# Zain-Jiang/Speech-Editing-Toolkit

Measured on AMD Instinct MI355X. Metric: diffusion mel-frames/s (100-step p_sample, B=32/GPU, T=800), higher is better.
Workload: dtype f32 (operands carried as 2 fp16 pieces, 3 MFMA products per term, fp32 accumulate: fp32-equivalent, see roofline.note)

## Files before the change

include/set_amd.h:

```cpp
#ifndef SET_AMD_H
#define SET_AMD_H

#include <stdint.h>

#ifdef __cplusplus
extern "C" {
#endif

#define SET_AMD_ABI_VERSION 2

#define SET_OK 0
#define SET_E_INVALID (-1)
#define SET_E_UNSUPPORTED (-2)
#define SET_E_LAUNCH (-3)

#define SET_ACT_NONE 0
#define SET_ACT_RELU 1
#define SET_ACT_GELU 2
#define SET_ACT_TANH 3
#define SET_ACT_SOFTPLUS 4
#define SET_ACT_MISH 5
#define SET_ACT_LRELU 6

#define SET_PRO_NONE 0
// ... 236 lines not shown
    uint16_t *y16;
    uint16_t *z16;
    int64_t d_bs, d_cs;
    int32_t B, T, dil, first;
} SetDiffnetLayerBf16Args;
int64_t set_sizeof_diffnet_layer_bf16_args(void);
int64_t set_diffnet_layer_bf16_image_size(void);
int set_pack_diffnet_layer_bf16(const float *wdil , const float *wcond ,
                                const float *wout , void *img, void *stream);
int set_pack_diffnet_layers_bf16(const float *wdil, const float *wcond, const float *wout, int64_t sdil, int64_t scond, int64_t sout,
                                 void *img, int32_t L, void *stream);
int set_diffnet_layer_fwd_bf16(const SetDiffnetLayerBf16Args *args, void *stream);
typedef struct SetDiffnetLayersBf16Args {
    const float *x_in;
    float *x_out;
    float *skip;
    const float *cond;
    const float *dstep;
    const void *img;
    const float *b_dil, *b_cond, *b_out;
    float *scratch;
    int64_t scratch_floats;
    int64_t d_bs, d_cs, d_ls;
    int32_t B, T, l0, nl, dilation_cycle_length, first;
} SetDiffnetLayersBf16Args;
int64_t set_sizeof_diffnet_layers_bf16_args(void);
int64_t set_diffnet_layers_bf16_scratch_floats(int32_t B, int32_t T, int32_t l0, int32_t nl, int32_t dilation_cycle_length);
int32_t set_diffnet_layers_bf16_plan(int32_t B, int32_t T, int32_t L, int32_t dilation_cycle_length);
int set_diffnet_layers_fwd_bf16(const SetDiffnetLayersBf16Args *args, void *stream);
int set_debug_bf16_phase_buffer(uint64_t *buf);
int set_debug_split_phase_buffer(uint64_t *buf);
int set_debug_x3_phase_buffer(uint64_t *buf);
int set_debug_resblock_phase_buffer(uint64_t *buf);

typedef struct SetDiffnetLayerBf16BwdArgs {
    const float *dx_out;
    const float *dskip;
    const uint16_t *y16;
    const void *img;
    float *dx;
    uint16_t *dy16;
    uint16_t *do16;
    float *dcond;
    float *part_dbo;
    float *part_dby;
    float *part_dd;
    int32_t B, T, dil, dcond_first;
} SetDiffnetLayerBf16BwdArgs;
int64_t set_sizeof_diffnet_layer_bf16_bwd_args(void);
int32_t set_diffnet_layer_bwd_bf16_tiles(int32_t T, int32_t dil);
int set_diffnet_layer_bwd_bf16(const SetDiffnetLayerBf16BwdArgs *args, void *stream);
int set_diffnet_layer_bwd_reduce(const float *part_dbo, const float *part_dby, const float *part_dd, int32_t B, int32_t tiles,
                                 float *db_out, float *db_dil, float *db_cond, float *dd, int64_t dd_bs, void *stream);
int set_diffnet_layers_bwd_reduce(const float *part_dbo, const float *part_dby, const float *part_dd, int32_t B, int32_t tiles, int32_t L,
                                  float *db_out, int64_t s_out, float *db_dil, int64_t s_dil, float *db_cond, int64_t s_cond, float *dd,
                                  int64_t dd_bs, int64_t dd_ls, void *stream);
int set_partial_rows_sum(const float *part, float *out, int32_t groups, int32_t rows, int32_t cols, int32_t accumulate,
                         float scale, void *stream);

int set_step_proj_fwd(const float *h, const float *w, int64_t w_ls, const float *b, int64_t b_ls, float *out, int32_t L, int32_t C,
                      int32_t N, void *stream);
int64_t set_step_proj_bwd_scratch_floats(int32_t L, int32_t C, int32_t N);
int set_step_proj_bwd(const float *h, const float *g, const float *w, int64_t w_ls, float *dh, float *dw, int64_t dw_ls, float *db,
                      int64_t db_ls, float *scratch, int32_t L, int32_t C, int32_t N, void *stream);
int set_step_proj_bwd_dh(const float *g, const float *w, int64_t w_ls, float *dh, float *scratch, int32_t L, int32_t C, int32_t N,
                         void *stream);
// ... 144 lines not shown
```

speech-editing-toolkit_amd/_lib.py:

```python
import ctypes as C
import os
import shutil
import subprocess

_PKG = os.path.dirname(os.path.abspath(__file__))
_ROOT = os.path.dirname(_PKG)
CSRC = os.path.join(_PKG, "csrc")
INCLUDE = os.path.join(_ROOT, "include")
LIB_PATH = os.path.join(_PKG, "libset_amd.so")
_LIB_OVERRIDE = os.environ.get("SET_AMD_LIB")
SOURCES = ["conv1d.hip", "conv_x2.hip", "resblock_x2.hip", "glue.hip", "diffnet.hip", "diffnet_x3.hip", "boundary.hip", "diffusion_ops.hip", "diffusion_loop.hip",
           "train.hip", "attention.hip", "attention_fused.hip", "bf16.hip", "diffnet_bf16.hip", "stutter.hip"]
HIPCC_FLAGS = ["--offload-arch=gfx950", "-O3", "-std=c++17", "-fPIC", "-shared", "-ffp-contract=off"]

OK, E_INVALID, E_UNSUPPORTED, E_LAUNCH = 0, -1, -2, -3
ACT = dict(none=0, relu=1, gelu=2, tanh=3, softplus=4, mish=5, lrelu=6)
PRO = dict(none=0, lrelu=1, div=2)
IMPL_NAIVE, IMPL_MFMA, IMPL_MFMA2, IMPL_BF16, IMPL_F16X2, IMPL_FEWOUT = 1, 2, 3, 4, 5, 6
DTYPE_F32, DTYPE_BF16, DTYPE_BF16_G16, DTYPE_BF16_G16_X16 = 0, 1, 2, 3

c_f32p = C.POINTER(C.c_float)
c_i64p = C.POINTER(C.c_int64)


# ... 231 lines not shown
    "set_conv1d_wgrad": (C.c_int, [_V, _V, _V, _V, _I32, _I32, _I32, _I32, _I32, _I32, _I32, _I32, _I32, _F, _I32, _V]),
    "set_conv1d_wgrad_scratch_floats": (_I64, [_I32, _I32, _I32, _I32, _I32, _I32]),
    "set_conv1d_wgrad_det": (C.c_int, [_V, _V, _V, _V, _I32, _I32, _I32, _I32, _I32, _I32, _I32, _I32, _I32, _F, _I32, _V, _I64, _V]),
    "set_conv1d_wgrad_grouped_scratch_floats": (_I64, [_I32, _I32, _I32, _I32, _I32, _I32]),
    "set_conv1d_wgrad_det_grouped": (C.c_int, [_V, _V, _V, _V, _I32, _I64, _I64, _I64, _I64, _I32, _I32, _I32, _I32, _I32, _I32, _I32, _I32,
                                               _I32, _V, _I64, _V]),
    "set_packed_conv_weight_bf16_size": (_I64, [_I32, _I32, _I32]),
    "set_pack_conv_weight_bf16": (C.c_int, [_V, _V, _I32, _I32, _I32, _I64, _I64, _I64, _I64, _V]),
    "set_sizeof_pack_bf16_desc": (_I64, []),
    "set_pack_conv_weights_bf16_batch": (C.c_int, [_V, _I32, _I64, _V]),
    "set_sizeof_pack_f32_desc": (_I64, []),
    "set_fill_pack_f32_desc": (_I64, [C.POINTER(SetPackF32Desc), _I32, _I32]),
    "set_pack_conv_weights_f32_batch": (C.c_int, [_V, _I32, _I64, _V]),
    "set_channel_sum_det": (C.c_int, [_V, _V, _I32, _I32, _I32, _V, _V]),
    "set_weighted_sum_det": (C.c_int, [_V, _V, _V, _I64, _I64, _V, _V]),
    "set_sumsq_det": (C.c_int, [_V, _V, _I64, _V, _V]),
    "set_dur_loss_sums_det": (C.c_int, [_V, _V, _V, _V, _V, _I32, _I32, _I32, _I32, _V, _V]),
    "set_pitch_loss_sums_det": (C.c_int, [_V, _V, _V, _V, _V, _I32, _I32, _V, _V]),
    "set_scatter_rows_segments": (_I32, [_I32]),
    "set_scatter_rows_det": (C.c_int, [_V, _V, _V, _I32, _I32, _I32, _I32, _F, _I32, _I32, _V, _V]),
    "set_sizeof_diffnet_layer_bf16_args": (_I64, []),
    "set_diffnet_layer_bf16_image_size": (_I64, []),
    "set_pack_diffnet_layer_bf16": (C.c_int, [_V, _V, _V, _V, _V]),
    "set_pack_diffnet_layers_bf16": (C.c_int, [_V, _V, _V, _I64, _I64, _I64, _V, _I32, _V]),
    "set_diffnet_layer_fwd_bf16": (C.c_int, [C.POINTER(SetDiffnetLayerBf16Args), _V]),
    "set_sizeof_diffnet_layers_bf16_args": (_I64, []),
    "set_diffnet_layers_bf16_scratch_floats": (_I64, [_I32, _I32, _I32, _I32, _I32]),
    "set_diffnet_layers_fwd_bf16": (C.c_int, [C.POINTER(SetDiffnetLayersBf16Args), _V]),
    "set_diffnet_layers_bf16_plan": (_I32, [_I32, _I32, _I32, _I32]),
    "set_debug_bf16_phase_buffer": (C.c_int, [_V]),
    "set_debug_split_phase_buffer": (C.c_int, [_V]),
    "set_debug_x3_phase_buffer": (C.c_int, [_V]),
    "set_debug_resblock_phase_buffer": (C.c_int, [_V]),
    "set_sizeof_diffnet_layer_bf16_bwd_args": (_I64, []),
    "set_diffnet_layer_bwd_bf16_tiles": (_I32, [_I32, _I32]),
    "set_diffnet_layer_bwd_bf16": (C.c_int, [C.POINTER(SetDiffnetLayerBf16BwdArgs), _V]),
    "set_partial_rows_sum": (C.c_int, [_V, _V, _I32, _I32, _I32, _I32, _F, _V]),
    "set_step_proj_fwd": (C.c_int, [_V, _V, _I64, _V, _I64, _V, _I32, _I32, _I32, _V]),
    "set_step_proj_bwd_scratch_floats": (_I64, [_I32, _I32, _I32]),
    "set_step_proj_bwd": (C.c_int, [_V, _V, _V, _I64, _V, _V, _I64, _V, _I64, _V, _I32, _I32, _I32, _V]),
    "set_step_proj_bwd_dh": (C.c_int, [_V, _V, _I64, _V, _V, _I32, _I32, _I32, _V]),
    "set_step_proj_bwd_dw": (C.c_int, [_V, _V, _V, _I64, _V, _I64, _I32, _I32, _I32, _V]),
    "set_diffnet_layer_bwd_reduce": (C.c_int, [_V, _V, _V, _I32, _I32, _V, _V, _V, _V, _I64, _V]),
    "set_diffnet_layers_bwd_reduce": (C.c_int, [_V, _V, _V, _I32, _I32, _I32, _V, _I64, _V, _I64, _V, _I64, _V, _I64, _I64, _V]),
    "set_channel_sum": (C.c_int, [_V, _V, _I32, _I32, _I32, _V]),
    "set_row_sum": (C.c_int, [_V, _V, _I64, _I32, _F, _V]),
    "set_conv_epilogue_bwd": (C.c_int, [_V, _V, _V, _V, _I32, _I32, _I32, _I32, _F, _V]),
    "set_act_fwd": (C.c_int, [_V, _V, _I64, _I32, _F, _V]),
    "set_act_bwd": (C.c_int, [_V, _V, _V, _I64, _I32, _F, _V]),
    "set_act_bwd_scaled": (C.c_int, [_V, _V, _V, _I64, _I32, _F, _F, _V]),
    "set_gate_bwd": (C.c_int, [_V, _V, _V, _I32, _I32, _I32, _V]),
    "set_res_skip_bwd": (C.c_int, [_V, _V, _V, _V, _I32, _I32, _I32, _V]),
    "set_layernorm_ch_bwd": (C.c_int, [_V, _V, _V, _V, _V, _V, _V, _V, _I32, _I32, _I32, _F, _V]),
    "set_layernorm_ch_bwd_add": (C.c_int, [_V, _V, _V, _V, _V, _V, _V, _V, _V, _I32, _I32, _I32, _F, _V]),
    "set_layernorm_ch_bwd_scratch": (C.c_int64, [_I32, _I32, _I32]),
    "set_embedding_bwd": (C.c_int, [_V, _V, _V, _I32, _I32, _I32, _I32, _F, _I32, _V]),
    "set_expand_states_bwd": (C.c_int, [_V, _V, _V, _I32, _I32, _I32, _I32, _V]),
    "set_dropout": (C.c_int, [_V, _V, _I64, _F, _U64, _U64, _V]),
    "set_residual_dropout": (C.c_int, [_V, _V, _V, _V, _I32, _I32, _I32, _F, _U64, _U64, _V]),
    "set_conv_epilogue_bwd_dropout": (C.c_int, [_V, _V, _V, _V, _I32, _I32, _I32, _F, _U64, _U64, _V]),
    "set_stutter_head_scratch_floats": (_I64, [_I32, _I32, _I32]),
    "set_stutter_head_loss": (C.c_int, [_V, _V, _V, _V, _V, _V, _V, _I32, _I32, _I32, _V]),
    "set_stutter_head_loss_bwd": (C.c_int, [_V, _V, _V, _V, _V, _V, _V, _V, _V, _V, _V, _I32, _I32, _I32, _V]),
    "set_stutter_head_bwd_reduce": (C.c_int, [_V, _V, _V, _I32, _I32, _I32, _V]),
    "set_frame_weight": (C.c_int, [_V, _V, _I64, _I32, _V]),
    "set_weighted_sum": (C.c_int, [_V, _V, _V, _I64, _I64, _V]),
# ... 114 lines not shown
```

speech-editing-toolkit_amd/csrc/boundary.hip:

```cpp
#include <stdlib.h>

#include "common.h"
#include "boundary_x2.h"
#include "diffnet_host.h"

namespace {
constexpr int DC = 256;
}

struct BoundaryArgs {
    const float *skip;
    float *x;
    const float *eps;
    const float *coef4;
    const float *w_skip_p, *b_skip, *w_outp_p, *b_outp, *w_in_p, *b_in;
    float *xin_next;
    float inv_div;
    float div;
    uint64_t seed, quad_offset;
    int T, M, MP;
};
constexpr int BD_LD = 64;

__global__ void __launch_bounds__(256, 2) diffnet_boundary_kernel(BoundaryArgs a) {
// ... 101 lines not shown
        const float *bp = smem + half * BD_LD + l31;
        gemm_groups<1, 2, 4>(acc[i], wp, bp, 2 * BD_LD, (a.MP / 2) / 4, [&](int) {
            wp += 4 * 64;
            bp += 4 * 2 * BD_LD;
        });
    }
    const rsrc_t ro = make_rsrc(a.xin_next + (int64_t)b * DC * T);
    float bin[2][16];
#pragma unroll
    for (int i = 0; i < 2; ++i)
#pragma unroll
        for (int r = 0; r < 16; ++r) bin[i][r] = (a.b_in + 32 * (2 * w + i) + urow16(r))[4 * half];
#pragma unroll
    for (int cb = 0; cb < 2; ++cb) {
        if (t0 + 32 * cb + l31 < T) {
            const unsigned so = 4u * (unsigned)(4 * half * T + t0 + 32 * cb + l31);
#pragma unroll
            for (int i = 0; i < 2; ++i)
#pragma unroll
                for (int r = 0; r < 16; ++r) {
                    const int ur = 32 * (2 * w + i) + urow16(r);
                    buf_store(fmaxf(acc[i][0][cb][r] + bin[i][r], 0.0f), ro, so, 4u * (unsigned)ur * (unsigned)T);
                }
        }
    }
}

struct BoundaryX2Args {
    BoundaryArgs g;
    const unsigned short *w_skip_x2, *w_outp_x2, *w_in_x2;
    int32_t *err_flag;
};

__global__ void __launch_bounds__(256, 2) diffnet_boundary_x2_kernel(BoundaryX2Args ax) {
    const BoundaryArgs &a = ax.g;
    extern __shared__ __attribute__((aligned(16))) unsigned char bl[];
    const int tid = threadIdx.x, lane = tid & 63;
    const int w = __builtin_amdgcn_readfirstlane(tid >> 6);
    const int half = lane >> 5, l31 = lane & 31;
    const int b = blockIdx.y, t0 = blockIdx.x * 64, T = a.T, M = a.M;
    const unsigned lane16 = 16u * (unsigned)lane;
    const unsigned T4 = 4u * (unsigned)T;
    float amax = 0.0f;
    {
        const int f = lane, cg = w;
        const rsrc_t rs = make_rsrc(a.skip + (int64_t)b * DC * T);
        const unsigned vo = 4u * (unsigned)min(t0 + f, T - 1);
        const bool tv = t0 + f < T;
        for (int c0 = 0; c0 < 64; c0 += 16) {
            float v[16];
#pragma unroll
            for (int u = 0; u < 16; ++u) v[u] = buf_load(rs, vo, (unsigned)(64 * cg + c0 + u) * T4);
#pragma unroll
            for (int q8 = 0; q8 < 2; ++q8) {
                bx_u32x4 u0, u1;
#pragma unroll
                for (int e = 0; e < 4; ++e) {
                    unsigned short p0[2], p1[2];
#pragma unroll
                    for (int k = 0; k < 2; ++k) {
                        const float sv = v[8 * q8 + 2 * e + k] / a.div;
                        const float x = tv ? sv : 0.0f;
                        amax = fmaxf(amax, fabsf(x));
                        bx_split(x, p0[k], p1[k]);
                    }
                    u0[e] = (unsigned)p0[0] | ((unsigned)p0[1] << 16);
                    u1[e] = (unsigned)p1[0] | ((unsigned)p1[1] << 16);
                }
                *reinterpret_cast<bx_u32x4 *>(bl + f * BX_XR + (64 * cg + c0 + 8 * q8) * 2) = u0;
                *reinterpret_cast<bx_u32x4 *>(bl + BX_PIECE + f * BX_XR + (64 * cg + c0 + 8 * q8) * 2) = u1;
            }
        }
    }
    __syncthreads();
    auto bfrag256 = [&](int ks, int cb) { return (unsigned)((cb * 32 + l31) * BX_XR + (ks * 16 + half * 8) * 2); };
    {
        const rsrc_t rw = make_rsrc(ax.w_skip_x2);
        const float inv = reinterpret_cast<const float *>(ax.w_skip_x2 + (DC / 32) * (DC / 16) * 1024)[1];
        f32x16 acc[2][2];
#pragma unroll
        for (int i = 0; i < 2; ++i)
#pragma unroll
            for (int cb = 0; cb < 2; ++cb) acc[i][cb] = (f32x16){0};
        bx_gemm<2>(acc, rw, lane16, 2 * w, DC / 16, DC / 16, bl, BX_PIECE, bfrag256);
        __syncthreads();
#pragma unroll
        for (int i = 0; i < 2; ++i)
#pragma unroll
            for (int cb = 0; cb < 2; ++cb)
#pragma unroll
                for (int g = 0; g < 4; ++g) {
                    unsigned short p0[4], p1[4];
#pragma unroll
                    for (int e = 0; e < 4; ++e) {
                        const int row = 32 * (2 * w + i) + 8 * g + 4 * half + e;
                        const float h = fmaxf(acc[i][cb][4 * g + e] * inv + a.b_skip[row], 0.0f);
                        amax = fmaxf(amax, h);
                        bx_split(h, p0[e], p1[e]);
                    }
                    const unsigned off = (unsigned)((cb * 32 + l31) * BX_XR + (32 * (2 * w + i) + 8 * g + 4 * half) * 2);
                    bx_u32x2 u;
                    u[0] = (unsigned)p0[0] | ((unsigned)p0[1] << 16); u[1] = (unsigned)p0[2] | ((unsigned)p0[3] << 16);
                    *reinterpret_cast<bx_u32x2 *>(bl + off) = u;
                    u[0] = (unsigned)p1[0] | ((unsigned)p1[1] << 16); u[1] = (unsigned)p1[2] | ((unsigned)p1[3] << 16);
                    *reinterpret_cast<bx_u32x2 *>(bl + BX_PIECE + off) = u;
                }
    }
    __syncthreads();
    float *xs = reinterpret_cast<float *>(bl);
    {
        const int rbn = (M + 31) / 32;
        f32x16 xo[1][2];
        xo[0][0] = (f32x16){0};
        xo[0][1] = (f32x16){0};
        const float inv = reinterpret_cast<const float *>(ax.w_outp_x2 + ((M + 31) / 32) * (DC / 16) * 1024)[1];
        if (w < rbn) bx_gemm<1>(xo, make_rsrc(ax.w_outp_x2), lane16, w, DC / 16, DC / 16, bl, BX_PIECE, bfrag256);
        __syncthreads();
        if (w < 3) {
#pragma unroll
            for (int r = 0; r < 16; ++r) {
                const int row = 32 * w + mfma32_row(r, lane);
                const float bias = a.b_outp[min(row, M - 1)];
#pragma unroll
                for (int cb = 0; cb < 2; ++cb) xs[row * 64 + 32 * cb + l31] = (w < rbn && row < M) ? xo[0][cb][r] * inv + bias : 0.0f;
            }
        }
    }
    __syncthreads();
    {
        const float c1 = a.coef4[0], c2 = a.coef4[1], sig = a.coef4[3] * expf(0.5f * a.coef4[2]);
        float *xb = a.x + (int64_t)b * M * T;
        const float *eb = a.eps ? a.eps + (int64_t)b * M * T : nullptr;
        for (int qi = tid; qi < 96 * 16; qi += 256) {
            const int m = qi >> 4, tq = qi & 15, t = t0 + 4 * tq;
            float *cell = xs + m * 64 + 4 * tq;
            if (m < M && t < T) {
                const int64_t i = (int64_t)m * T + t;
                const f32x4 xt = *reinterpret_cast<const f32x4 *>(xb + i);
                float z[4];
                if (eb) {
                    const f32x4 e4 = *reinterpret_cast<const f32x4 *>(eb + i);
                    z[0] = e4[0]; z[1] = e4[1]; z[2] = e4[2]; z[3] = e4[3];
                } else {
                    randn4(a.seed, a.quad_offset + (uint64_t)(((int64_t)b * M * T + i) >> 2), z);
                }
                f32x4 o;
#pragma unroll
                for (int k = 0; k < 4; ++k) {
                    const float mean = c1 * cell[k] + c2 * xt[k];
                    o[k] = mean + sig * z[k];
                }
                *reinterpret_cast<f32x4 *>(xb + i) = o;
                *reinterpret_cast<f32x4 *>(cell) = o;
            } else {
                *reinterpret_cast<f32x4 *>(cell) = (f32x4){0.0f, 0.0f, 0.0f, 0.0f};
            }
        }
    }
    if (!a.xin_next) {
        if (!(amax < 32768.0f) && ax.err_flag) __hip_atomic_store(ax.err_flag, 2, __ATOMIC_RELAXED, __HIP_MEMORY_SCOPE_AGENT);
        return;
    }
    __syncthreads();
    unsigned char *xp = bl + BX_PIECE;
    constexpr unsigned XP_PIECE = 64 * BX_PR;
    {
        const int f = lane, cg = w;
#pragma unroll
        for (int q8 = 0; q8 < 3; ++q8) {
            bx_u32x4 u0, u1;
#pragma unroll
            for (int e = 0; e < 4; ++e) {
                unsigned short p0[2], p1[2];
#pragma unroll
                for (int k = 0; k < 2; ++k) {
                    const float x = xs[(24 * cg + 8 * q8 + 2 * e + k) * 64 + f];
                    amax = fmaxf(amax, fabsf(x));
                    bx_split(x, p0[k], p1[k]);
                }
                u0[e] = (unsigned)p0[0] | ((unsigned)p0[1] << 16);
                u1[e] = (unsigned)p1[0] | ((unsigned)p1[1] << 16);
            }
            *reinterpret_cast<bx_u32x4 *>(xp + f * BX_PR + (24 * cg + 8 * q8) * 2) = u0;
            *reinterpret_cast<bx_u32x4 *>(xp + XP_PIECE + f * BX_PR + (24 * cg + 8 * q8) * 2) = u1;
        }
    }
    if (!(amax < 32768.0f) && ax.err_flag) __hip_atomic_store(ax.err_flag, 2, __ATOMIC_RELAXED, __HIP_MEMORY_SCOPE_AGENT);
    __syncthreads();
    {
        const int ngin = ((M + 31) / 32) * 2;
        const float inv = reinterpret_cast<const float *>(ax.w_in_x2 + (DC / 32) * ngin * 1024)[1];
        f32x16 acc[2][2];
#pragma unroll
        for (int i = 0; i < 2; ++i)
#pragma unroll
            for (int cb = 0; cb < 2; ++cb) acc[i][cb] = (f32x16){0};
        bx_gemm<2>(acc, make_rsrc(ax.w_in_x2), lane16, 2 * w, ngin, ngin, xp, XP_PIECE,
                   [&](int ks, int cb) { return (unsigned)((cb * 32 + l31) * BX_PR + (ks * 16 + half * 8) * 2); });
        const rsrc_t ro = make_rsrc(a.xin_next + (int64_t)b * DC * T);
        float bin[2][16];
#pragma unroll
        for (int i = 0; i < 2; ++i)
#pragma unroll
            for (int r = 0; r < 16; ++r) bin[i][r] = (a.b_in + 32 * (2 * w + i) + urow16(r))[4 * half];
#pragma unroll
        for (int cb = 0; cb < 2; ++cb) {
            if (t0 + 32 * cb + l31 < T) {
                const unsigned so = 4u * (unsigned)(4 * half * T + t0 + 32 * cb + l31);
#pragma unroll
                for (int i = 0; i < 2; ++i)
#pragma unroll
                    for (int r = 0; r < 16; ++r) {
                        const int ur = 32 * (2 * w + i) + urow16(r);
                        buf_store(fmaxf(acc[i][cb][r] * inv + bin[i][r], 0.0f), ro, so, 4u * (unsigned)ur * (unsigned)T);
                    }
            }
        }
    }
}

bool boundary_fusable(const SetDiffLoopArgs &a) {
    if (const char *e = getenv("SET_AMD_FUSED_BOUNDARY"))
        if (atoi(e) == 0) return false;
    return a.T % 4 == 0 && a.M <= 96 && a.M >= 2 && ((a.M + 15) / 16 * 16 / 2) % 8 == 0;
}

int launch_boundary(const SetDiffLoopArgs &a, int Bg, const float *skip, float *x, const float *eps, int sid, uint64_t quad_offset,
                    float *xin_next, bool x2, hipStream_t s) {
    static SetDeviceOnce lds_once;
    if (int rc = set_lds_optin(lds_once, 80 * 1024, "boundary(attr)", diffnet_boundary_kernel, diffnet_boundary_x2_kernel)) return rc;
    BoundaryArgs g = {};
    g.skip = skip; g.x = x; g.eps = eps; g.coef4 = a.coef4 + 4 * sid;
    g.w_skip_p = a.w_skip_p; g.b_skip = a.b_skip; g.w_outp_p = a.w_outp_p; g.b_outp = a.b_outp;
    g.w_in_p = a.w_in_p; g.b_in = a.b_in; g.xin_next = xin_next;
    g.div = sqrtf((float)a.L); g.seed = a.seed; g.quad_offset = quad_offset;
    g.T = a.T; g.M = a.M; g.MP = (a.M + 15) / 16 * 16;
    if (x2) {
        BoundaryX2Args gx = {};
        gx.g = g;
        gx.w_skip_x2 = reinterpret_cast<const unsigned short *>(a.w_skip_x2);
        gx.w_outp_x2 = reinterpret_cast<const unsigned short *>(a.w_outp_x2);
        gx.w_in_x2 = reinterpret_cast<const unsigned short *>(a.w_in_x2);
        gx.err_flag = a.err_flag;
        hipLaunchKernelGGL(diffnet_boundary_x2_kernel, dim3((a.T + 63) / 64, Bg), dim3(256), (size_t)2 * BX_PIECE, s, gx);
    } else {
        hipLaunchKernelGGL(diffnet_boundary_kernel, dim3((a.T + 63) / 64, Bg), dim3(256), (size_t)DC * BD_LD * sizeof(float), s, g);
    }
    return set_check_launch("set_diffusion_loop(boundary)");
}
```

speech-editing-toolkit_amd/csrc/conv_x2.hip:

```cpp
#include <stdlib.h>

#include <type_traits>

#include "common.h"

typedef _Float16 cx_f16x8 __attribute__((ext_vector_type(8)));
typedef unsigned cx_u32x4 __attribute__((ext_vector_type(4)));

__device__ int g_x2_range_flag = 0;

namespace {

constexpr int CX_KCH = 32;
constexpr int CX_ROWB = CX_KCH * 2 + 16;

template <int N> using cx_ic = std::integral_constant<int, N>;

__device__ __forceinline__ unsigned short cx_f2h(float x) { return __builtin_bit_cast(unsigned short, (_Float16)x); }
__device__ __forceinline__ float cx_h2f(unsigned short u) { return (float)__builtin_bit_cast(_Float16, u); }
__device__ __forceinline__ f32x16 cx_mma(cx_u32x4 a, cx_u32x4 b, f32x16 c) {
    return __builtin_amdgcn_mfma_f32_32x32x16_f16(__builtin_bit_cast(cx_f16x8, a), __builtin_bit_cast(cx_f16x8, b), c, 0, 0, 0);
}
__device__ __forceinline__ cx_u32x4 cx_load_u4(rsrc_t r, unsigned voff, unsigned soff) {
    return __builtin_amdgcn_raw_buffer_load_b128(r, (int)voff, (int)soff, 0);
}
template <int PRO>
__device__ __forceinline__ float cx_pro(float v, float p) {
    if constexpr (PRO == SET_PRO_LRELU) return v > 0.0f ? v : v * p;
    else if constexpr (PRO == SET_PRO_DIV) return v / p;
    else return v;
}
static inline int cx_round_up(int x, int m) { return (x + m - 1) / m * m; }

__global__ void __launch_bounds__(256) pack_conv_x2_kernel(const float *w, unsigned short *img, int Cout, int Cin, int K, int CoutP,
                                                           int CinP, int64_t n_frag_elems, int64_t w_base, int64_t w_sco,
                                                           int64_t w_sci, int64_t w_stap, float scale, int phases, int kfull) {
// ... 279 lines not shown
            if (has_div) y = y / a.out_div;
            buf_store(y, d_out, (tv && row < a.Cout) ? (ro[r] * (unsigned)a.out_cs + (unsigned)nc) * 4u : BUF_OOB, 0u);
        }
    };
    auto finish = [&](auto ACT) __attribute__((always_inline)) {
#pragma unroll
        for (int i = 0; i < RBW; ++i) {
            if (r0 + (wm * RBW + i) * 32 >= a.Cout) continue;
#pragma unroll
            for (int j = 0; j < NCB; ++j) tile(ACT, acc[i][j], i, j);
        }
    };
    switch (a.act) {
        case SET_ACT_NONE: finish(cx_ic<SET_ACT_NONE>{}); break;
        case SET_ACT_RELU: finish(cx_ic<SET_ACT_RELU>{}); break;
        case SET_ACT_LRELU: finish(cx_ic<SET_ACT_LRELU>{}); break;
        default: finish(cx_ic<-1>{}); break;
    }
}

template <int WM, int WN, int RBW, int NCB, bool PHASES = false>
int launch_conv_x2(const SetConv1dArgs &a, int lo, int halo, hipStream_t s, int ph_u = 0, int ph_pad = 0) {
    constexpr int MB = 32 * RBW * WM, NB = 32 * NCB * WN;
    const int CinP = cx_round_up(a.Cin, CX_KCH), CoutP = cx_round_up(a.Cout, 32);
    const size_t lds = (size_t)2 * (NB + halo) * CX_ROWB;
    static SetDeviceOnce lds_once;
    if (int rc = set_lds_optin(lds_once, 96 * 1024, "conv x2 attr", conv1d_x2_kernel<WM, WN, RBW, NCB, PHASES>)) return rc;
    if (lds > 96 * 1024) return set_fail(SET_E_UNSUPPORTED, "set_conv1d(f16x2)", "tile does not fit LDS");
    dim3 grid((a.T_iter + NB - 1) / NB, (a.Cout + MB - 1) / MB, a.B), block(256);
    hipLaunchKernelGGL((conv1d_x2_kernel<WM, WN, RBW, NCB, PHASES>), grid, block, lds, s, a, lo, halo, CinP, CoutP, ph_u, ph_pad);
    return set_check_launch("set_conv1d(f16x2)");
}

}

extern "C" int64_t set_packed_conv_weight_x2_size(int32_t Cout, int32_t Cin, int32_t K) {
    return (int64_t)2 * (cx_round_up(Cout, 32) / 32) * (cx_round_up(Cin, CX_KCH) / 16) * K * 512 + 8;
}

static int pack_x2(const float *w, void *wp, int Cout, int Cin, int K, int64_t w_base, int64_t w_sco, int64_t w_sci, int64_t w_stap,
                   int scale_exp, int phases, int kfull, void *stream, const char *what) {
    SET_REQUIRE(w && wp && Cout > 0 && Cin > 0 && K > 0 && scale_exp >= -60 && scale_exp <= 60, what);
    const int CoutP = cx_round_up(Cout, 32), CinP = cx_round_up(Cin, CX_KCH);
    const int64_t n = (int64_t)(CoutP / 32) * (CinP / 16) * K * 512;
    hipLaunchKernelGGL(pack_conv_x2_kernel, dim3(set_blocks(n, 256)), dim3(256), 0, (hipStream_t)stream, w,
                       reinterpret_cast<unsigned short *>(wp), Cout, Cin, K, CoutP, CinP, n, w_base, w_sco, w_sci, w_stap,
                       ldexpf(1.0f, scale_exp), phases, kfull);
    return set_check_launch(what);
}

extern "C" int set_pack_conv_weight_x2(const float *w, void *wp, int32_t Cout, int32_t Cin, int32_t K, int64_t w_base, int64_t w_sco,
                                       int64_t w_sci, int64_t w_stap, int32_t scale_exp, void *stream) {
    return pack_x2(w, wp, Cout, Cin, K, w_base, w_sco, w_sci, w_stap, scale_exp, 0, 0, stream, "set_pack_conv_weight_x2");
}

extern "C" int64_t set_packed_conv_transpose_x2_size(int32_t Cout, int32_t Cin, int32_t k, int32_t u) {
    return set_packed_conv_weight_x2_size(Cout * u, Cin, (k + u - 1) / u);
}
extern "C" int set_pack_conv_transpose_x2(const float *w, void *wp, int32_t Cout, int32_t Cin, int32_t k, int32_t u, int32_t scale_exp,
                                          void *stream) {
    SET_REQUIRE(u >= 1 && k >= u, "set_pack_conv_transpose_x2");
    return pack_x2(w, wp, Cout * u, Cin, (k + u - 1) / u, 0, 0, 0, 0, scale_exp, u, k, stream, "set_pack_conv_transpose_x2");
}

extern "C" int set_conv_transpose1d_x2(const float *in, const void *wp, const float *bias, float *out, int32_t B, int32_t Cin,
                                       int32_t Cout, int32_t k, int32_t u, int32_t P, int32_t T_in, int32_t pro, float pro_param,
// ... 9 lines not shown
    SET_REQUIRE(a.T_out > 0, "set_conv_transpose1d_x2");
    if (((int64_t)Cout * a.T_out) * 4 >= ((int64_t)1 << 31) || ((int64_t)Cin * T_in) * 4 >= ((int64_t)1 << 31))
        return set_fail(SET_E_UNSUPPORTED, "set_conv_transpose1d_x2", "one batch slice of in / out exceeds 2 GiB");
    const int lo = -(J - 1), halo = J - 1;
    hipStream_t s = (hipStream_t)stream;
    if (a.Cout > 64) return launch_conv_x2<4, 1, 1, 4, true>(a, lo, halo, s, u, P);
    return launch_conv_x2<2, 2, 1, 4, true>(a, lo, halo, s, u, P);
}

int set_resblock_pair_range_flag_(int *flag, int reset);

extern "C" int set_conv_x2_range_flag(int32_t *flag, int32_t reset) {
    int v = 0, vp = 0;
    SET_HIP(hipMemcpyFromSymbol(&v, HIP_SYMBOL(g_x2_range_flag), sizeof(int)), "set_conv_x2_range_flag");
    if (int rc = set_resblock_pair_range_flag_(&vp, reset)) return rc;
    if (flag) *flag = v | vp;
    if (reset && v) {
        const int z = 0;
        SET_HIP(hipMemcpyToSymbol(HIP_SYMBOL(g_x2_range_flag), &z, sizeof(int)), "set_conv_x2_range_flag");
    }
    return SET_OK;
}

int set_conv1d_x2_dispatch(const SetConv1dArgs &a, hipStream_t s) {
    if (a.in_chan_add) return set_fail(SET_E_UNSUPPORTED, "set_conv1d(f16x2)", "per-channel add is an fp32 / bf16 path");
    const int o_first = -a.pad, o_last = (a.K - 1) * a.dil - a.pad;
    const int lo = o_first < o_last ? o_first : o_last;
    const int halo = (o_first < o_last ? o_last : o_first) - lo;
    if (halo > 128) return set_fail(SET_E_UNSUPPORTED, "set_conv1d(f16x2)", "receptive field > 128");
    const int64_t cs = a.res && a.res_cs > a.out_cs ? a.res_cs : a.out_cs;
    if (((int64_t)cx_round_up(a.Cout, 32) * cs + a.T_out) * 4 >= ((int64_t)1 << 31) ||
        ((int64_t)a.Cin * a.in_cs + a.T_in) * 4 >= ((int64_t)1 << 31))
        return set_fail(SET_E_UNSUPPORTED, "set_conv1d(f16x2)", "one batch slice of in / out / res exceeds 2 GiB");
    if (a.Cout > 64) return launch_conv_x2<4, 1, 1, 4>(a, lo, halo, s);
    if (a.Cout > 32) return launch_conv_x2<2, 2, 1, 4>(a, lo, halo, s);
    return launch_conv_x2<1, 4, 1, 2>(a, lo, halo, s);
}
```

speech-editing-toolkit_amd/diffnet.py:

```python
import math
import os

import torch
from torch import nn

from . import autograd_ops, ops
from .hparams import hparams as _global_hparams


def _kaiming_conv1d(cin, cout, k, **kw):
    layer = nn.Conv1d(cin, cout, k, **kw)
    nn.init.kaiming_normal_(layer.weight)
    return layer


class ResidualBlock(nn.Module):

    def __init__(self, encoder_hidden, residual_channels, dilation):
        super().__init__()
        C = residual_channels
        self.dilation = dilation
        self.dilated_conv = _kaiming_conv1d(C, 2 * C, 3, padding=dilation, dilation=dilation)
        self.diffusion_projection = nn.Linear(C, C)
        self.conditioner_projection = _kaiming_conv1d(encoder_hidden, 2 * C, 1)
# ... 115 lines not shown
                                                                      ops._stream()), "set_pack_diffnet_layer_bf16")
            row = img.stride(0) * img.element_size()
            return img, [(img.data_ptr() + i * row, ps[6 * i + 3].data_ptr(), ps[6 * i + 1].data_ptr(), ps[6 * i + 5].data_ptr(),
                          int(ly.dilation)) for i, ly in enumerate(layers)]
        return self._img16.get(key, build)

    def step_table(self, t_values):
        C, L = self.C, self.n_layers
        n = t_values.numel()
        emb = ops.sinusoid_embed(t_values, C).view(1, C, n)
        h = ops.conv1d(emb, self._w_mlp0, self.mlp[0].bias, act="mish")
        h = ops.conv1d(h, self._w_mlp2, self.mlp[2].bias)
        out = torch.empty(1, L * C, n, dtype=torch.float32, device=h.device)
        for l, layer in enumerate(self.residual_layers):
            ops.conv1d(h, layer._w_dproj, layer.diffusion_projection.bias, out=out[:, l * C:(l + 1) * C, :])
        return out.view(L * C, n)

    def step_table_all(self, steps, dev):
        ps = [self.mlp[0].weight, self.mlp[0].bias, self.mlp[2].weight, self.mlp[2].bias]
        for layer in self.residual_layers:
            ps += [layer.diffusion_projection.weight, layer.diffusion_projection.bias]

        def build(_):
            prev = ops.compute_dtype()
            ops.set_compute_dtype("f32")
            try:
                return self.step_table(torch.arange(int(steps), device=dev).to(torch.float32))
            finally:
                ops.set_compute_dtype(prev)
        if torch.is_grad_enabled():
            return build(None)
        return self._dtab.get(ops.weights_key(ps, int(steps), str(dev), ops._DEFAULT_IMPL), build)

    def cond_projections(self, cond):
        B, H, T = cond.shape
        C, L = self.C, self.n_layers
        out = torch.empty(B, L * 2 * C, T, dtype=torch.float32, device=cond.device)
        if not torch.is_grad_enabled():
            ps = [t for layer in self.residual_layers for t in (layer.conditioner_projection.weight, layer.conditioner_projection.bias)]

            def build(_):
                w_all = torch.cat([p.detach() for p in ps[0::2]], 0).contiguous()
                return ops.ConvWeight(w_all, L * 2 * C, H, 1), torch.cat([p.detach() for p in ps[1::2]], 0).contiguous()
            cw, b_all = self._cond_all.get(ops.weights_key(ps, str(cond.device)), build)
            ops.conv1d(cond, cw, b_all, out=out)
            return out
        for l, layer in enumerate(self.residual_layers):
            ops.conv1d(cond, layer._w_cond, layer.conditioner_projection.bias,
                       out=out[:, l * 2 * C:(l + 1) * 2 * C, :])
        return out

    def denoise(self, x, condproj, dtab, col, batch_cols):
        B, M, T = x.shape
        C, L = self.C, self.n_layers
        n = dtab.shape[1]
        fused = self.use_fused()
        h = ops.conv1d(x, self._w_in, self.input_projection.bias, act="relu")
        skip = torch.empty(B, C, T, dtype=torch.float32, device=x.device)
        nxt = torch.empty_like(h)
        for l, layer in enumerate(self.residual_layers):
            cp = condproj[:, l * 2 * C:(l + 1) * 2 * C, :]
            if fused:
                w1p, w2p = layer.fused_weights()
                dptr = dtab.data_ptr() + 4 * (l * C * n + col)
                ops.diffnet_layer(h, cp.data_ptr(), condproj.stride(0), dptr, 1 if batch_cols else 0, n,
                                  w1p, layer.dilated_conv.bias, w2p, layer.output_projection.bias,
                                  nxt, skip, layer.dilation, l == 0)
                h, nxt = nxt, h
            else:
                d = dtab.view(L, C, n)[l]
                d = d[:, col:col + B].t().contiguous() if batch_cols else d[:, col].reshape(1, C).expand(B, C).contiguous()
                y = ops.conv1d(h, layer._w_dil, layer.dilated_conv.bias, dil=layer.dilation,
                               pad=layer.dilation, in_chan_add=d, res=cp)
                z = ops.gate(y)
                o = ops.conv1d(z, layer._w_out, layer.output_projection.bias)
                h = ops.res_skip(h, o, skip, l == 0)
        hs = ops.conv1d(skip, self._w_skip, self.skip_projection.bias, pro="div", pro_param=math.sqrt(L),
                        act="relu")
# ... 56 lines not shown
```

speech-editing-toolkit_amd/ops.py:

```python
import collections
import ctypes as C
import math
import os
import typing

import torch

from . import _lib
from ._lib import (ACT, PRO, IMPL_BF16, IMPL_MFMA, IMPL_MFMA2, IMPL_NAIVE, SetConv1dArgs, SetDiffnetLayerArgs,
                   SetDiffLoopArgs, SetDiffnetStackArgs, check)

_DEFAULT_IMPL = os.environ.get("SET_AMD_CONV_IMPL", "auto")
_WEIGHTS_EPOCH = 0


_COMPUTE_DTYPE = os.environ.get("SET_AMD_DTYPE", "f32")


def set_compute_dtype(dtype):
    global _COMPUTE_DTYPE
    if dtype not in ("f32", "bf16"):
        raise ValueError("compute dtype must be 'f32' or 'bf16', got %r" % (dtype,))
    _COMPUTE_DTYPE = dtype

# ... 228 lines not shown
            registry.add(self)
        return wp

    def packed(self):
        w = self.raw()
        self._used32 = True
        return self._img32.get(weights_key((w,)), lambda wp: self._pack(w, wp, "conv_weight", torch.float32, _F32_IMAGES))

    def packed_bf16(self):
        w = self.raw()
        return self._img16.get(weights_key((w,)), lambda wp: self._pack(w, wp, "conv_weight_bf16", torch.bfloat16, _BF16_IMAGES))

    def packed_x2(self):
        w = self.raw()
        return self._img_x2.get(weights_key((w,)), lambda _: self._pack(w, None, "conv_weight_x2", torch.float16, tail=(_x2_exponent(w),)))

    def packed_v2(self, dil):
        w = self.raw()
        halo = (self.K - 1) * abs(dil)
        slot = 128 if (64 + halo) * 256 * 4 > 96 * 1024 else 256
        wp, _ = self._img2.setdefault(slot, CacheSlot()).get(weights_key((w,)), lambda old: (
            self._pack(w, old and old[0], "conv_weight_v2", torch.float32, _F32_IMAGES, mid=(int(dil),)), int(dil)))
        self._used2.add(slot)
        return wp


def _x2_exponent(w):
    m = float(w.abs().max())
    return max(-60, min(60, 4 - math.frexp(m)[1])) if m > 0 and math.isfinite(m) else 0


def f16x2_eligible(T_iter, Cout, Cin, K, dil):
    return T_iter >= 64 and Cout >= 32 and Cin >= 32 and K >= 2 and Cin * K >= 96 and (K - 1) * abs(dil) <= 128


def conv_x2_range_flag(reset=True):
    v = C.c_int32(0)
    check(_lib.lib().set_conv_x2_range_flag(C.byref(v), int(bool(reset))), "set_conv_x2_range_flag")
    return bool(v.value)


def bf16_eligible(T_iter, Cout, Cin, K, dil, out_stride=1, out_off=0):
    return (T_iter >= 32 and Cout >= 32 and Cin * K >= 64 and out_stride == 1 and out_off == 0
            and (K - 1) * abs(dil) <= 128)


_AUTO_SPLIT = [False]


class split_convs:

    def __init__(self, on=True):
        self.on = bool(on)

    def __enter__(self):
        self.prev, _AUTO_SPLIT[0] = _AUTO_SPLIT[0], self.on

    def __exit__(self, *exc):
        _AUTO_SPLIT[0] = self.prev


def _pick_impl(impl, T_iter, Cout=0, Cin=0, K=1, dil=1, out_stride=1, out_off=0, chan_add=False, plain=False, pad=0):
    impl = impl or _DEFAULT_IMPL
    if impl == "auto":
        if T_iter < 16:
            return "naive"
# ... 808 lines not shown
```

speech-editing-toolkit_amd/spec_denoiser.py:

```python
from functools import partial

import numpy as np
import torch
from torch import nn

from . import autograd_ops, ops
from .diffusion_utils import get_noise_schedule_list
from .fs import FastSpeech, FastSpeechNormal, MelEncoder
from .hparams import hparams as _global_hparams


class GaussianDiffusion(nn.Module):
    fs_cls = FastSpeech
    unused_parameter_prefixes = ("fs.decoder.", "fs.mel_out.")

    def __init__(self, phone_encoder, out_dims, denoise_fn, timesteps=1000, time_scale=1, loss_type="l1",
                 betas=None, spec_min=None, spec_max=None, hp=None):
        super().__init__()
        hp = hp if hp is not None else _global_hparams
        self.hp = hp
        self.denoise_fn = denoise_fn
        self.fs = self.fs_cls(len(phone_encoder), hp)
        self.mel_encoder = MelEncoder(hidden_size=self.fs.hidden_size)
        self.mel_bins = out_dims
# ... 97 lines not shown
        x0 = F.add_chan_mask(x0.contiguous(), None, tgt_nonpad)
        ret["mel_out_bct"] = x0
        ret["mel_out"] = F.bct_to_btc(x0)
        ret["x_t"] = x_t
        ret["t"] = t
        return ret

    def _forward_infer(self, txt_tokens, time_mel_masks, mel2ph, spk_embed, ref_mels, f0, uv, use_pred_mel2ph,
                       use_pred_pitch, noises, seed, want_layer_spans, n_groups, persistent):
        ret, cond = self.conditioner(txt_tokens, time_mel_masks, mel2ph, spk_embed, ref_mels, f0, uv, True,
                                     use_pred_mel2ph, use_pred_pitch)
        ret.pop("tgt_nonpad")
        ret.pop("pitch_pred_bct", None)
        B, H, T = cond.shape
        M = self.mel_bins
        dev = cond.device
        dn = self.denoise_fn
        steps = self.num_timesteps
        seed = int(seed) if seed is not None else int(torch.randint(0, 2 ** 31 - 1, (1,)).item())
        if noises is not None:
            noises = noises.reshape(steps + 1, B, M, T).contiguous()
            x = noises[0].clone()
            eps = noises[1:]
        else:
            x = ops.randn((B, M, T), dev, seed, 0)
            eps = None
        ids = torch.arange(steps, device=dev)
        coef4 = self.posterior_coef(ids)
        dtab = dn.step_table_all(steps, dev)
        bf16 = None
        if ops.compute_dtype() == "bf16" and dn.use_fused() and dn.encoder_hidden == 192 and T >= 32:
            bf16 = dict(cond=cond.contiguous(), imgs=dn.bf16_layer_images()[0],
                        b_cond=torch.stack([l.conditioner_projection.bias for l in dn.residual_layers]).contiguous())
        condproj = dn.cond_projections(cond) if bf16 is None else None
        if dn.use_fused():
            def loop():
                return ops.diffusion_loop(
                    x=x, noise=eps, seed=seed, condproj=condproj, dstep=dtab, coef4=coef4, bf16=bf16,
                    w_in=dn._w_in, b_in=dn.input_projection.bias,
                    packs=dn.fused_packs(),
                    w_skip=dn._w_skip, b_skip=dn.skip_projection.bias,
                    w_outp=dn._w_outp, b_outp=dn.output_projection.bias,
                    L=dn.n_layers, steps=steps, dilation_cycle_length=dn.dilation_cycle_length,
                    want_layer_spans=want_layer_spans, n_groups=n_groups, persistent=persistent)
            x_T = x.clone()
            try:
                spans = loop()
            except ops.SplitRangeError:
                import warnings
                warnings.warn("spec_denoiser: activation outside the fp16 split range; repeating the reverse loop with the "
                              "bf16x3 splitting")
                x.copy_(x_T)
                with ops.split_operand_mode_as(3):
                    spans = loop()
            if spans is not None:
                ret.update(spans)
        else:
            quads = (B * M * T + 3) // 4
            for k, i in enumerate(reversed(range(steps))):
                x0 = dn.denoise(x, condproj, dtab, i, False)
                ops.posterior_step(x0, x, coef4[i:i + 1], eps=None if eps is None else eps[k], out=x, seed=seed,
                                   offset=(k + 1) * quads)
        ret["mel_out"] = ops.bct_to_btc(x)
        ret["cond"] = cond
        return ret


class GaussianDiffusionNormal(GaussianDiffusion):
    fs_cls = FastSpeechNormal

    def conditioner(self, txt_tokens, time_mel_masks, mel2ph, spk_embed, ref_mels, f0, uv, infer=False,
                    use_pred_mel2ph=False, use_pred_pitch=False, dropout_seed=0):
        if use_pred_mel2ph or use_pred_pitch:
            raise TypeError("spec_denoiser_normal.GaussianDiffusion.forward has no use_pred_mel2ph / use_pred_pitch")
        F = autograd_ops if torch.is_grad_enabled() else ops
        ret = self.fs(txt_tokens, mel2ph, spk_embed, f0, uv, None, skip_decoder=True, infer=infer,
                      dropout_seed=dropout_seed)
        B, T, M = ref_mels.shape
        tmask = time_mel_masks.reshape(B, T).contiguous()
        masked = ops.mul_one_minus_mask(ref_mels.contiguous(), tmask, M)
        cond = self.mel_encoder.run(ops.btc_to_bct(masked), res=ret.pop("decoder_inp_bct"), mask=ret["tgt_nonpad"])
        ret["decoder_inp"] = F.bct_to_btc(cond)
        return ret, cond
```

Before: 178,100.

## Route conditioner 1x1 projection through fp16x2-split MFMA kernel, add boundary probe

Adds a dedicated pointwise projection kernel that splits fp32 activations into two fp16 pieces in LDS and runs the packed-weight MFMA GEMM, with a split over output row blocks. The all-layer conditioner projection in the sampling path now uses it by default when the fp16 split mode is active, in place of the general conv path. It adds a range flag and a fallback that redoes the projection in fp32 and reruns the loop if the conditioner overflows the fp16 split range. It also adds an optional compile-time timestamp probe in the boundary kernel, off by default.

New measurement: 179,300 (median of 6 runs). About the same (+0.7%).

```diff
diff --git a/include/set_amd.h b/include/set_amd.h
--- a/include/set_amd.h
+++ b/include/set_amd.h
@@ -292,6 +292,7 @@
 int set_debug_split_phase_buffer(uint64_t *buf);
 int set_debug_x3_phase_buffer(uint64_t *buf);
 int set_debug_resblock_phase_buffer(uint64_t *buf);
+int set_debug_boundary_timeline(uint64_t *host_ticks);
 
 typedef struct SetDiffnetLayerBf16BwdArgs {
     const float *dx_out;
diff --git a/speech-editing-toolkit_amd/_lib.py b/speech-editing-toolkit_amd/_lib.py
--- a/speech-editing-toolkit_amd/_lib.py
+++ b/speech-editing-toolkit_amd/_lib.py
@@ -287,6 +287,7 @@
     "set_debug_split_phase_buffer": (C.c_int, [_V]),
     "set_debug_x3_phase_buffer": (C.c_int, [_V]),
     "set_debug_resblock_phase_buffer": (C.c_int, [_V]),
+    "set_debug_boundary_timeline": (C.c_int, [C.POINTER(C.c_uint64)]),
     "set_sizeof_diffnet_layer_bf16_bwd_args": (_I64, []),
     "set_diffnet_layer_bwd_bf16_tiles": (_I32, [_I32, _I32]),
     "set_diffnet_layer_bwd_bf16": (C.c_int, [C.POINTER(SetDiffnetLayerBf16BwdArgs), _V]),
diff --git a/speech-editing-toolkit_amd/csrc/boundary.hip b/speech-editing-toolkit_amd/csrc/boundary.hip
--- a/speech-editing-toolkit_amd/csrc/boundary.hip
+++ b/speech-editing-toolkit_amd/csrc/boundary.hip
@@ -157,7 +157,22 @@
     int32_t *err_flag;
 };
 
+#ifndef SET_BX_PROBE
+#define SET_BX_PROBE 0
+#endif
+__device__ uint64_t g_bx_timeline[16];
+#if SET_BX_PROBE
+#define BX_TS(k) { __builtin_amdgcn_sched_barrier(0); ts[k] = __builtin_amdgcn_s_memtime(); __builtin_amdgcn_sched_barrier(0); }
+#define BX_TS_OUT if (blockIdx.x == 1 && blockIdx.y == 1 && threadIdx.x == 0) { for (int k = 0; k < 10; ++k) g_bx_timeline[k] = ts[k]; }
+#else
+#define BX_TS(k)
+#define BX_TS_OUT
+#endif
 __global__ void __launch_bounds__(256, 2) diffnet_boundary_x2_kernel(BoundaryX2Args ax) {
+#if SET_BX_PROBE
+    uint64_t ts[10] = {};
+#endif
+    BX_TS(0)
     const BoundaryArgs &a = ax.g;
     extern __shared__ __attribute__((aligned(16))) unsigned char bl[];
     const int tid = threadIdx.x, lane = tid & 63;
@@ -198,6 +213,7 @@
         }
     }
     __syncthreads();
+    BX_TS(2)
     auto bfrag256 = [&](int ks, int cb) { return (unsigned)((cb * 32 + l31) * BX_XR + (ks * 16 + half * 8) * 2); };
     {
         const rsrc_t rw = make_rsrc(ax.w_skip_x2);
@@ -208,6 +224,7 @@
 #pragma unroll
             for (int cb = 0; cb < 2; ++cb) acc[i][cb] = (f32x16){0};
         bx_gemm<2>(acc, rw, lane16, 2 * w, DC / 16, DC / 16, bl, BX_PIECE, bfrag256);
+        BX_TS(3)
         __syncthreads();
 #pragma unroll
         for (int i = 0; i < 2; ++i)
@@ -232,6 +249,7 @@
                 }
     }
     __syncthreads();
+    BX_TS(4)
     float *xs = reinterpret_cast<float *>(bl);
     {
         const int rbn = (M + 31) / 32;
@@ -240,6 +258,7 @@
         xo[0][1] = (f32x16){0};
         const float inv = reinterpret_cast<const float *>(ax.w_outp_x2 + ((M + 31) / 32) * (DC / 16) * 1024)[1];
         if (w < rbn) bx_gemm<1>(xo, make_rsrc(ax.w_outp_x2), lane16, w, DC / 16, DC / 16, bl, BX_PIECE, bfrag256);
+        BX_TS(5)
         __syncthreads();
         if (w < 3) {
 #pragma unroll
@@ -252,6 +271,7 @@
         }
     }
     __syncthreads();
+    BX_TS(6)
     {
         const float c1 = a.coef4[0], c2 = a.coef4[1], sig = a.coef4[3] * expf(0.5f * a.coef4[2]);
         float *xb = a.x + (int64_t)b * M * T;
@@ -287,6 +307,7 @@
         return;
     }
     __syncthreads();
+    BX_TS(7)
     unsigned char *xp = bl + BX_PIECE;
     constexpr unsigned XP_PIECE = 64 * BX_PR;
     {
@@ -312,6 +333,7 @@
     }
     if (!(amax < 32768.0f) && ax.err_flag) __hip_atomic_store(ax.err_flag, 2, __ATOMIC_RELAXED, __HIP_MEMORY_SCOPE_AGENT);
     __syncthreads();
+    BX_TS(8)
     {
         const int ngin = ((M + 31) / 32) * 2;
         const float inv = reinterpret_cast<const float *>(ax.w_in_x2 + (DC / 32) * ngin * 1024)[1];
@@ -342,6 +364,14 @@
             }
         }
     }
+    BX_TS(9)
+    BX_TS_OUT
+}
+
+extern "C" int set_debug_boundary_timeline(uint64_t *host_ticks) {
+    SET_REQUIRE(host_ticks, "set_debug_boundary_timeline");
+    SET_HIP(hipMemcpyFromSymbol(host_ticks, HIP_SYMBOL(g_bx_timeline), 10 * sizeof(uint64_t)), "set_debug_boundary_timeline");
+    return SET_OK;
 }
 
 bool boundary_fusable(const SetDiffLoopArgs &a) {
diff --git a/speech-editing-toolkit_amd/csrc/conv_x2.hip b/speech-editing-toolkit_amd/csrc/conv_x2.hip
--- a/speech-editing-toolkit_amd/csrc/conv_x2.hip
+++ b/speech-editing-toolkit_amd/csrc/conv_x2.hip
@@ -2,6 +2,7 @@
 
 #include <type_traits>
 
+#include "boundary_x2.h"
 #include "common.h"
 
 typedef _Float16 cx_f16x8 __attribute__((ext_vector_type(8)));
@@ -347,6 +348,120 @@
     return set_check_launch("set_conv1d(f16x2)");
 }
 
+template <int NRB, bool NT>
+__global__ void __launch_bounds__(256, 2) proj_x2_kernel(const float *x, const unsigned short *wimg, const float *bias, float *out, int64_t in_bs,
+                                                          int64_t in_cs, int64_t out_bs, int64_t out_cs, int Cin, int Cout, int T, int ng16, int upb) {
+    extern __shared__ __attribute__((aligned(16))) unsigned char pl[];
+    const int tid = threadIdx.x, lane = tid & 63;
+    const int w = __builtin_amdgcn_readfirstlane(tid >> 6);
+    const int half = lane >> 5, l31 = lane & 31;
+    const int t0 = blockIdx.x * 64, b = blockIdx.y;
+    const unsigned XR = (unsigned)Cin * 2u + 16u, piece_bytes = 64u * XR;
+    {
+        const rsrc_t rx = make_rsrc(x + (int64_t)b * in_bs);
+        const unsigned vo = 4u * (unsigned)min(t0 + lane, T - 1);
+        const bool tv = t0 + lane < T;
+        const int n_oct = Cin / 8;
+        float amax = 0.0f;
+        for (int o0 = w; o0 < n_oct; o0 += 12) {
+            float v[3][8];
+#pragma unroll
+            for (int j = 0; j < 3; ++j) {
+                const int o = min(o0 + 4 * j, n_oct - 1);
+#pragma unroll
+                for (int e = 0; e < 8; ++e) v[j][e] = buf_load(rx, vo, (unsigned)((8 * o + e) * (int)in_cs) * 4u);
+            }
+#pragma unroll
+            for (int j = 0; j < 3; ++j) {
+                const int o = o0 + 4 * j;
+                if (o < n_oct) {
+                    cx_u32x4 u0, u1;
+#pragma unroll
+                    for (int k = 0; k < 4; ++k) {
+                        const float v0 = tv ? v[j][2 * k] : 0.0f, v1 = tv ? v[j][2 * k + 1] : 0.0f;
+                        amax = fmaxf(fmaxf(amax, fabsf(v0)), fabsf(v1));
+                        unsigned p0, p1;
+                        split2_f16(v0, v1, p0, p1);
+                        u0[k] = p0; u1[k] = p1;
+                    }
+                    *reinterpret_cast<cx_u32x4 *>(pl + lane * XR + o * 16) = u0;
+                    *reinterpret_cast<cx_u32x4 *>(pl + piece_bytes + lane * XR + o * 16) = u1;
+                }
+            }
+        }
+        if (!(amax < 32768.0f)) __hip_atomic_store(&g_x2_range_flag, 1, __ATOMIC_RELAXED, __HIP_MEMORY_SCOPE_AGENT);
+    }
+    __syncthreads();
+    const int nrb = Cout / 32, nks = Cin / 16;
+    const rsrc_t rw = make_rsrc(wimg);
+    const rsrc_t ro = make_rsrc(out + (int64_t)b * out_bs);
+    const rsrc_t rbias = make_rsrc(bias ? bias : out);
+    const float inv = reinterpret_cast<const float *>(wimg + (int64_t)nrb * ng16 * 1024)[1];
+    const unsigned lane16 = 16u * (unsigned)lane;
+    const unsigned row4 = (unsigned)out_cs * 4u;
+    auto bfrag = [&](int ks, int cb) { return (unsigned)(cb * 32 + l31) * XR + (unsigned)(ks * 16 + half * 8) * 2u; };
+    auto unit = [&](auto N, int rb0) __attribute__((always_inline)) {
+        constexpr int kN = decltype(N)::value;
+        f32x16 acc[kN][2];
+#pragma unroll
+        for (int i = 0; i < kN; ++i)
+#pragma unroll
+            for (int cb = 0; cb < 2; ++cb) acc[i][cb] = (f32x16){0};
+        bx_gemm<kN>(acc, rw, lane16, rb0, ng16, nks, pl, piece_bytes, bfrag);
+        float bz[kN][16];
+#pragma unroll
+        for (int i = 0; i < kN; ++i)
+#pragma unroll
+            for (int r = 0; r < 16; ++r) bz[i][r] = bias ? buf_load(rbias, 16u * (unsigned)half, 4u * (unsigned)(32 * (rb0 + i) + urow16(r))) : 0.0f;
+#pragma unroll
+        for (int cb = 0; cb < 2; ++cb) {
+            const int t = t0 + 32 * cb + l31;
+            if (t < T) {
+                const unsigned so = (unsigned)(4 * half) * row4 + 4u * (unsigned)t;
+#pragma unroll
+                for (int i = 0; i < kN; ++i)
+#pragma unroll
+                    for (int r = 0; r < 16; ++r)
+                        __builtin_amdgcn_raw_buffer_store_b32(__builtin_bit_cast(unsigned, acc[i][cb][r] * inv + bz[i][r]), ro, (int)so,
+                                                              (int)((unsigned)(32 * (rb0 + i) + urow16(r)) * row4), NT ? 2 : 0);
+            }
+        }
+    };
+    const int n_units = (nrb + NRB - 1) / NRB;
+    const int u_end = min(n_units, ((int)blockIdx.z + 1) * upb);
+    for (int u = (int)blockIdx.z * upb + w; u < u_end; u += 4) {
+        const int rb0 = u * NRB;
+        if (rb0 + NRB <= nrb) {
+            unit(cx_ic<NRB>{}, rb0);
+        } else {
+            for (int rb = rb0; rb < nrb; ++rb) unit(cx_ic<1>{}, rb);
+        }
+    }
+}
+
+bool proj_x2_takes(const SetConv1dArgs &a) {
+    return a.K == 1 && a.pad == 0 && !a.res && !a.mask && !a.in_chan_add && !a.accumulate && a.pro == SET_PRO_NONE && a.act == SET_ACT_NONE &&
+           a.alpha == 1.0f && a.out_stride == 1 && a.out_off == 0 && a.T_iter == a.T_in && a.T_out == a.T_in && a.out_cs == a.T_out &&
+           a.Cin % 16 == 0 && a.Cin <= 256 && a.Cout % 32 == 0 && a.T_iter >= 64;
+}
+
+template <int NRB, bool NT>
+int launch_proj_x2(const SetConv1dArgs &a, hipStream_t s) {
+    static SetDeviceOnce lds_once;
+    if (int rc = set_lds_optin(lds_once, 80 * 1024, "proj x2 attr", proj_x2_kernel<NRB, NT>)) return rc;
+    const int ntiles = (a.T_iter + 63) / 64, n_units = (a.Cout / 32 + NRB - 1) / NRB;
+    const int64_t tiles = (int64_t)ntiles * a.B;
+    int nsplit = (int)((4096 + tiles - 1) / tiles);
+    nsplit = max(1, min(nsplit, (n_units + 7) / 8));
+    const int upb = (n_units + nsplit - 1) / nsplit;
+    nsplit = (n_units + upb - 1) / upb;
+    if (a.B > 65535 || nsplit > 65535) return set_fail(SET_E_UNSUPPORTED, "set_conv1d(f16x2)", "grid too large");
+    const size_t lds = (size_t)2 * 64 * (a.Cin * 2 + 16);
+    hipLaunchKernelGGL((proj_x2_kernel<NRB, NT>), dim3(ntiles, a.B, nsplit), dim3(256), lds, s, a.in, reinterpret_cast<const unsigned short *>(a.w),
+                       a.bias, a.out, a.in_bs, a.in_cs, a.out_bs, a.out_cs, a.Cin, a.Cout, a.T_iter, cx_round_up(a.Cin, CX_KCH) / 16, upb);
+    return set_check_launch("set_conv1d(f16x2 projection)");
+}
+
 }
 
 extern "C" int64_t set_packed_conv_weight_x2_size(int32_t Cout, int32_t Cin, int32_t K) {
@@ -422,6 +537,11 @@
     if (((int64_t)cx_round_up(a.Cout, 32) * cs + a.T_out) * 4 >= ((int64_t)1 << 31) ||
         ((int64_t)a.Cin * a.in_cs + a.T_in) * 4 >= ((int64_t)1 << 31))
         return set_fail(SET_E_UNSUPPORTED, "set_conv1d(f16x2)", "one batch slice of in / out / res exceeds 2 GiB");
+#ifndef SET_PROJ_X2_NRB
+#define SET_PROJ_X2_NRB 2
+#define SET_PROJ_X2_NT 1
+#endif
+    if (proj_x2_takes(a)) return launch_proj_x2<SET_PROJ_X2_NRB, SET_PROJ_X2_NT != 0>(a, s);
     if (a.Cout > 64) return launch_conv_x2<4, 1, 1, 4>(a, lo, halo, s);
     if (a.Cout > 32) return launch_conv_x2<2, 2, 1, 4>(a, lo, halo, s);
     return launch_conv_x2<1, 4, 1, 2>(a, lo, halo, s);
diff --git a/speech-editing-toolkit_amd/diffnet.py b/speech-editing-toolkit_amd/diffnet.py
--- a/speech-editing-toolkit_amd/diffnet.py
+++ b/speech-editing-toolkit_amd/diffnet.py
@@ -171,7 +171,7 @@
             return build(None)
         return self._dtab.get(ops.weights_key(ps, int(steps), str(dev), ops._DEFAULT_IMPL), build)
 
-    def cond_projections(self, cond):
+    def cond_projections(self, cond, x2=False):
         B, H, T = cond.shape
         C, L = self.C, self.n_layers
         out = torch.empty(B, L * 2 * C, T, dtype=torch.float32, device=cond.device)
@@ -182,7 +182,7 @@
                 w_all = torch.cat([p.detach() for p in ps[0::2]], 0).contiguous()
                 return ops.ConvWeight(w_all, L * 2 * C, H, 1), torch.cat([p.detach() for p in ps[1::2]], 0).contiguous()
             cw, b_all = self._cond_all.get(ops.weights_key(ps, str(cond.device)), build)
-            ops.conv1d(cond, cw, b_all, out=out)
+            ops.conv1d(cond, cw, b_all, out=out, impl="f16x2" if x2 and ops.proj_x2_eligible(T, L * 2 * C, H, out) else None)
             return out
         for l, layer in enumerate(self.residual_layers):
             ops.conv1d(cond, layer._w_cond, layer.conditioner_projection.bias,
diff --git a/speech-editing-toolkit_amd/ops.py b/speech-editing-toolkit_amd/ops.py
--- a/speech-editing-toolkit_amd/ops.py
+++ b/speech-editing-toolkit_amd/ops.py
@@ -284,6 +284,15 @@
 
 def f16x2_eligible(T_iter, Cout, Cin, K, dil):
     return T_iter >= 64 and Cout >= 32 and Cin >= 32 and K >= 2 and Cin * K >= 96 and (K - 1) * abs(dil) <= 128
+
+
+def proj_x2_eligible(T, Cout, Cin, out=None):
+    return T >= 64 and Cin % 16 == 0 and 16 <= Cin <= 256 and Cout % 32 == 0 and Cout >= 32 and (out is None or out.is_contiguous())
+
+
+def proj_x2_selected():
+    return (os.environ.get("SET_AMD_PROJ_X2", "1") != "0" and os.environ.get("SET_AMD_X3", "1") != "0" and split_operand_mode() == 2
+            and _COMPUTE_DTYPE == "f32" and _DEFAULT_IMPL == "auto")
 
 
 def conv_x2_range_flag(reset=True):
diff --git a/speech-editing-toolkit_amd/spec_denoiser.py b/speech-editing-toolkit_amd/spec_denoiser.py
--- a/speech-editing-toolkit_amd/spec_denoiser.py
+++ b/speech-editing-toolkit_amd/spec_denoiser.py
@@ -153,7 +153,8 @@
         if ops.compute_dtype() == "bf16" and dn.use_fused() and dn.encoder_hidden == 192 and T >= 32:
             bf16 = dict(cond=cond.contiguous(), imgs=dn.bf16_layer_images()[0],
                         b_cond=torch.stack([l.conditioner_projection.bias for l in dn.residual_layers]).contiguous())
-        condproj = dn.cond_projections(cond) if bf16 is None else None
+        proj_x2 = bf16 is None and dn.use_fused() and ops.proj_x2_selected()
+        condproj = dn.cond_projections(cond, x2=proj_x2) if bf16 is None else None
         if dn.use_fused():
             def loop():
                 return ops.diffusion_loop(
@@ -174,6 +175,18 @@
                 x.copy_(x_T)
                 with ops.split_operand_mode_as(3):
                     spans = loop()
+            if proj_x2 and ops.conv_x2_range_flag(reset=True):
+                import warnings
+                warnings.warn("spec_denoiser: conditioner outside the fp16 split range; repeating the projection on the fp32 pipe "
+                              "and the reverse loop")
+                condproj = dn.cond_projections(cond)
+                x.copy_(x_T)
+                try:
+                    spans = loop()
+                except ops.SplitRangeError:
+                    x.copy_(x_T)
+                    with ops.split_operand_mode_as(3):
+                        spans = loop()
             if spans is not None:
                 ret.update(spans)
         else:
```
